# angelocatalani/neural-network-compression

Hardware: AMD Instinct MI355X
Metric: weights/sec through prune+k-means (K=256) (higher is better)
Workload: dtype f32

## Files before the change

neural_network_compression_amd/csrc/nnc_common.hpp:

```cpp
#pragma once
#include <hip/hip_runtime.h>
#include <hip/hip_ext.h>

#include <algorithm>
#include <atomic>
#include <chrono>
#include <mutex>
#include <cmath>
#include <cstdio>
#include <cstdlib>
#include <cstring>
#include <queue>
#include <string>
#include <vector>

#include "nnc.h"

int nnc_set_error_(int code, const char *msg);
int nnc_current_device_(void);
int nnc_cu_count_(void);
void nnc_prof_take_(int tag, hipEvent_t *a, hipEvent_t *b);

static inline int fail(int code, const std::string &msg) { return nnc_set_error_(code, msg.c_str()); }
static inline int current_device() { return nnc_current_device_(); }
static inline int cu_count() { return nnc_cu_count_(); }
static inline void prof_take(int tag, hipEvent_t *a, hipEvent_t *b) { nnc_prof_take_(tag, a, b); }
#define NNC_MAX_DEVICES 64

#define HIPCHK(expr)                                                                       \
    do {                                                                                   \
        hipError_t e_ = (expr);                                                            \
        if (e_ != hipSuccess)                                                              \
            return fail(NNC_EHIP, std::string(#expr) + ": " + hipGetErrorString(e_));      \
    } while (0)

#define LAUNCHCHK(name)                                                                    \
    do {                                                                                   \
        hipError_t e_ = hipGetLastError();                                                 \
        if (e_ != hipSuccess)                                                              \
            return fail(NNC_EHIP, std::string("launch ") + name + ": " + hipGetErrorString(e_)); \
    } while (0)

static inline hipStream_t S(void *stream) { return reinterpret_cast<hipStream_t>(stream); }

static inline int stream_grid(int64_t work_items, int threads, int per_cu)
{
    int64_t blocks = (work_items + threads - 1) / threads;
    int64_t cap = (int64_t)cu_count() * per_cu;
    if (blocks < 1) blocks = 1;
    return (int)std::min<int64_t>(blocks, cap);
}

#define NNC_LAUNCH_PROF(tag, kernel, grid, block, lds, stream, ...)                                   \
    do {                                                                                               \
        hipEvent_t ea_, eb_;                                                                           \
        prof_take(tag, &ea_, &eb_);                                                                    \
        hipExtLaunchKernelGGL(kernel, grid, block, lds, stream, ea_, eb_, 0, __VA_ARGS__);             \
    } while (0)

#define WAVE 64

__device__ __forceinline__ void wave_lds_fence()
{
    __builtin_amdgcn_fence(__ATOMIC_RELEASE, "wavefront");
    __builtin_amdgcn_wave_barrier();
    __builtin_amdgcn_fence(__ATOMIC_ACQUIRE, "wavefront");
}

#define LEAF 128
struct PwHeap { int start[256]; int len[256]; float val[256]; };


template <bool WAVE_ONLY = false, typename F>
__device__ float block_pairwise_sum(F elem, int n, PwHeap *hp)
{
    const int tid = threadIdx.x, nthr = blockDim.x;
    if (n <= LEAF) {
        if (tid < 8) {
            float res = 0.0f;
            if (n < 8) {
                for (int i = 0; i < n; i++) res += elem(i);
            } else {
                float r = elem(tid);
                const int lim = n - (n % 8);
                for (int i = 8; i < lim; i += 8) r += elem(i + tid);
                r = r + __shfl_xor(r, 1);
                r = r + __shfl_xor(r, 2);
                r = r + __shfl_xor(r, 4);
                res = r;
                for (int i = lim; i < n; i++) res += elem(i);
            }
            if (tid == 0) hp->val[1] = res;
        }
        if (WAVE_ONLY) wave_lds_fence();
        else __syncthreads();
        return hp->val[1];
    }
    for (int i = tid; i < 256; i += nthr) { hp->start[i] = 0; hp->len[i] = 0; hp->val[i] = 0.0f; }
    __syncthreads();
    if (tid == 0) { hp->start[1] = 0; hp->len[1] = n; }
    __syncthreads();
    int depth = 0;
    while (depth < 7 && ((n + (1 << depth) - 1) >> depth) > LEAF) depth++;
    if (depth < 7) depth++;
    for (int lev = 0; lev < depth; lev++) {
        const int i = (1 << lev) + tid;
        if (tid < (1 << lev)) {
            const int l = hp->len[i];
            if (l > LEAF) {
                int n2 = l / 2; n2 -= n2 % 8;
                hp->start[2 * i] = hp->start[i]; hp->len[2 * i] = n2;
                hp->start[2 * i + 1] = hp->start[i] + n2; hp->len[2 * i + 1] = l - n2;
            }
        }
        __syncthreads();
    }
    const int j = tid & 7;
    for (int node = 1 + (tid >> 3); node < (2 << depth) && node < 256; node += (nthr >> 3)) {
        const int l = hp->len[node];
        if (l > 0 && l <= LEAF) {
            const int st = hp->start[node];
            float res;
            if (l < 8) {
                res = 0.0f;
                for (int i = 0; i < l; i++) res += elem(st + i);
            } else {
                float r = elem(st + j);
                const int lim = l - (l % 8);
                for (int i = 8; i < lim; i += 8) r += elem(st + i + j);
                r = r + __shfl_xor(r, 1);
                r = r + __shfl_xor(r, 2);
                r = r + __shfl_xor(r, 4);
                res = r;
                for (int i = lim; i < l; i++) res += elem(st + i);
            }
            if (j == 0) hp->val[node] = res;
        }
    }
    __syncthreads();
    for (int lev = depth - 1; lev >= 0; lev--) {
        const int i = (1 << lev) + tid;
        if (tid < (1 << lev) && hp->len[i] > LEAF) hp->val[i] = hp->val[2 * i] + hp->val[2 * i + 1];
        __syncthreads();
    }
    return hp->val[1];
}

template <typename F>
__device__ float wave_pairwise_sum(F elem, int n, PwHeap *hp)
{
    const int lane = threadIdx.x & 63;
    if (n <= LEAF) {
        if (lane < 8) {
            float res = 0.0f;
            if (n < 8) {
                for (int i = 0; i < n; i++) res += elem(i);
            } else {
                float r = elem(lane);
                const int lim = n - (n % 8);
                for (int i = 8; i < lim; i += 8) r += elem(i + lane);
                r = r + __shfl_xor(r, 1);
                r = r + __shfl_xor(r, 2);
                r = r + __shfl_xor(r, 4);
                res = r;
                for (int i = lim; i < n; i++) res += elem(i);
            }
            if (lane == 0) hp->val[1] = res;
        }
        wave_lds_fence();
        return hp->val[1];
    }
    hp->start[lane] = 0; hp->len[lane] = 0; hp->val[lane] = 0.0f;
    wave_lds_fence();
    if (lane == 0) { hp->start[1] = 0; hp->len[1] = n; }
    wave_lds_fence();
    int depth = 0;
    while (depth < 5 && ((n + (1 << depth) - 1) >> depth) > LEAF) depth++;
    if (depth < 5) depth++;
    for (int lev = 0; lev < depth; lev++) {
        const int i = (1 << lev) + lane;
        if (lane < (1 << lev)) {
            const int l = hp->len[i];
            if (l > LEAF) {
                int n2 = l / 2; n2 -= n2 % 8;
                hp->start[2 * i] = hp->start[i]; hp->len[2 * i] = n2;
                hp->start[2 * i + 1] = hp->start[i] + n2; hp->len[2 * i + 1] = l - n2;
            }
        }
        wave_lds_fence();
    }
    const int j8 = lane & 7;
    for (int node = 1 + (lane >> 3); node < (2 << depth) && node < 64; node += 8) {
        const int l = hp->len[node];
        if (l > 0 && l <= LEAF) {
            const int st = hp->start[node];
            float res;
            if (l < 8) {
                res = 0.0f;
                for (int i = 0; i < l; i++) res += elem(st + i);
            } else {
                float r = elem(st + j8);
                const int lim = l - (l % 8);
                for (int i = 8; i < lim; i += 8) r += elem(st + i + j8);
                r = r + __shfl_xor(r, 1);
                r = r + __shfl_xor(r, 2);
                r = r + __shfl_xor(r, 4);
                res = r;
                for (int i = lim; i < l; i++) res += elem(st + i);
            }
            if (j8 == 0) hp->val[node] = res;
        }
    }
    wave_lds_fence();
    for (int lev = depth - 1; lev >= 0; lev--) {
        const int i = (1 << lev) + lane;
        if (lane < (1 << lev) && hp->len[i] > LEAF) hp->val[i] = hp->val[2 * i] + hp->val[2 * i + 1];
        wave_lds_fence();
    }
    return hp->val[1];
}
```

neural_network_compression_amd/csrc/nnc_hip.hip:

```cpp
#include "nnc_common.hpp"
#include "nnc_km_shared.hpp"


extern "C" size_t nnc_kmeans_workspace_bytes(int32_t k)
{
    (void)k;
    return sizeof(KmWs) + 256;
}

extern "C" int32_t nnc_fix_shift(float absmax, int64_t n_total)
{
    int L = 1;
    while (((int64_t)1 << L) < n_total && L < 62) L++;
    if (!(absmax > 0.0f) || !std::isfinite(absmax)) return 0;
    int P = 0;
    (void)std::frexp((double)absmax, &P);
    return std::min(28, 62 - L) - P;
}

__device__ __forceinline__ int fix_f32(float v, int Sft)
{
    return (int)rintf(ldexpf(v, Sft));
}

// ... 230 lines not shown
    if (MODE == 1 && n_dev) n = *n_dev;
    unsigned long long *trace = (MODE == 0) ? NNC_KM_TRACE_PTR : nullptr;
    unsigned long long tr0 = 0, tr1 = 0, tr2 = 0;
    if (trace) tr0 = __builtin_amdgcn_s_memrealtime();

    const int64_t nvec = VEC ? (n >> 2) : 0;
    const int64_t nsteps = nvec / KM_THREADS;
    const int64_t tails = DEAL ? (int64_t)(gridDim.x >> 1) : 0;
    const int64_t nmain = nsteps - 2 * tails;
    const int64_t per = (nmain + gridDim.x - 1) / gridDim.x;
    int64_t s0 = tails + (int64_t)blockIdx.x * per;
    const int64_t mend = nsteps - tails;
    if (s0 > mend) s0 = mend;
    const int64_t s1 = (s0 + per < mend) ? (s0 + per) : mend;
    const int64_t dealt = DEAL ? (((int64_t)blockIdx.x < tails) ? (int64_t)blockIdx.x : nsteps - 1 - ((int64_t)blockIdx.x - tails)) : 0;
    const int64_t count = (s1 - s0) + (DEAL ? 1 : 0);
    auto step_of = [&](int64_t kk) -> int64_t { return DEAL ? (kk == 0 ? dealt : s0 + kk - 1) : s0 + kk; };
    const float4 *x4 = reinterpret_cast<const float4 *>(x);
    const float4 *base = x4 + threadIdx.x;
#ifdef KM_NT_LOADS
    auto ld = [&](int64_t kk) -> float4 { return kk < count ? __builtin_nontemporal_load(&base[step_of(kk) * KM_THREADS]) : make_float4(0.f, 0.f, 0.f, 0.f); };
#else
    auto ld = [&](int64_t kk) -> float4 { return kk < count ? base[step_of(kk) * KM_THREADS] : make_float4(0.f, 0.f, 0.f, 0.f); };
#endif
    float4 r[KM_RING];
#pragma unroll
    for (int j = 0; j < KM_RING; j++) r[j] = ld(j);

    if (MODE == 0 && !(which & 2) && (ws->st.done | ws->st.paused)) return;
    if (MODE == 1 && n_dev && s0 >= s1 && blockIdx.x != gridDim.x - 1) return;
    const int k = ws->p.k;
    const int glog2 = ws->glog2, rlog2 = ws->rlog2;
    const int G = 1 << glog2;
    const int kp = (k + 7) & ~7;
    const int t = ws->cur ^ (which & 1);
    const KmTab *__restrict__ tab = &ws->tab[t];
#ifdef KM_KU_FAST
    const int kt = (which & 1) ? tab->ku : ws->ku_cur;
#else
    const int kt = tab->ku;
#endif

    uint16_t *cell_s = reinterpret_cast<uint16_t *>(smem);
    float4 *pair_s = reinterpret_cast<float4 *>(smem + ((size_t)2 << glog2));
    float *cval_s = reinterpret_cast<float *>(smem + ((size_t)2 << glog2) + (size_t)kp * 16);
    uint16_t *orig_s = reinterpret_cast<uint16_t *>(smem + ((size_t)2 << glog2) + (size_t)kp * 20);
    size_t off = (((size_t)2 << glog2) + (size_t)kp * 22 + 15) & ~(size_t)15;
    unsigned *ovf_s = reinterpret_cast<unsigned *>(smem + off);
    off += KM_OVF_MAX * 4;
    unsigned long long *sum_s = reinterpret_cast<unsigned long long *>(smem + off);
    unsigned *cnt_s = reinterpret_cast<unsigned *>(smem + off + ((size_t)k << rlog2) * 8);

    {
        const uint4 *src = reinterpret_cast<const uint4 *>(tab->cell);
        uint4 *dst = reinterpret_cast<uint4 *>(cell_s);
        for (int i = threadIdx.x; i < (G >> 3); i += KM_THREADS) dst[i] = src[i];
        for (int i = threadIdx.x; i < kt; i += KM_THREADS) {
            float2 a = tab->cand[i];
            float2 b = (i + 1 < kt) ? tab->cand[i + 1] : a;
            pair_s[i] = make_float4(a.x, a.y, b.x, b.y);
            cval_s[i] = a.x;
            orig_s[i] = tab->orig[i];
        }
        {
            const int novf = min(tab->n_ovf, KM_OVF_MAX);
            for (int i = threadIdx.x; i < novf; i += KM_THREADS) ovf_s[i] = tab->ovf[i];
        }
        if (MODE == 0) {
            const int tot = k << rlog2;
            for (int i = threadIdx.x; i < tot; i += KM_THREADS) { sum_s[i] = 0ull; cnt_s[i] = 0u; }
        }
        if (MODE == 1 && dist_hist) {
            unsigned *hz = reinterpret_cast<unsigned *>(sum_s);
            for (int i = threadIdx.x; i < 4096; i += KM_THREADS) hz[i] = 0u;
        }
    }
    __syncthreads();
    unsigned *hist_s = (MODE == 1 && dist_hist) ? reinterpret_cast<unsigned *>(sum_s) : nullptr;
    KmHistRun hr;
    hr.bin = 0xFFFFFFFFu; hr.cnt = 0;

    KmCtx c;
    c.cell_s = cell_s; c.pair_s = pair_s; c.cval_s = cval_s; c.orig_s = orig_s; c.ovf_s = ovf_s; c.sum_s = sum_s; c.cnt_s = cnt_s;
    c.mean = ws->p.x_mean; c.lo = ws->p.lo; c.inv = ws->inv;
    c.Sft = ws->p.fix_shift; c.gmax = G - 1; c.k = kt; c.rlog2 = rlog2;
    c.rep = threadIdx.x & ((1 << rlog2) - 1);
    KmRun run;
    run.p = -1; run.cnt = 0; run.sum = 0;
    if (trace) tr1 = __builtin_amdgcn_s_memrealtime();

    for (int64_t kk = 0; kk < count; kk += KM_RING) {
#pragma unroll
        for (int j = 0; j < KM_RING; j++) {
            const int64_t kcur = kk + j;
            const float4 v = r[j];
            r[j] = ld(kcur + KM_RING);
            if (kcur < count) {
                if (MODE == 0) km_accumulate4<ABL>(c, v, run);
                else {
                    const float xa[4] = {v.x, v.y, v.z, v.w};
                    km_emit<4, LT>(c, xa, 4 * (step_of(kcur) * KM_THREADS + threadIdx.x), labels_out, quant_out, dist_out, hist_s, hr);
                }
            }
        }
    }
    if (blockIdx.x == gridDim.x - 1) {
        const int64_t vdone = nsteps * KM_THREADS;
        {
            for (int64_t v = vdone + threadIdx.x; v < nvec; v += KM_THREADS) {
                const float4 a4 = x4[v];
                const float xa[4] = {a4.x, a4.y, a4.z, a4.w};
                if (MODE == 0) km_accumulate4<ABL>(c, a4, run);
                else km_emit<4, LT>(c, xa, 4 * v, labels_out, quant_out, dist_out, hist_s, hr);
            }
            for (int64_t i = (nvec << 2) + threadIdx.x; i < n; i += KM_THREADS) {
                const float xs[1] = {x[i]};
                if (MODE == 0) km_accumulate<1, ABL>(c, xs, run);
                else km_emit<1, LT>(c, xs, i, labels_out, quant_out, dist_out, hist_s, hr);
            }
        }
    }
    if (trace) tr2 = __builtin_amdgcn_s_memrealtime();
    if (MODE == 0) {
        if (ABL != 1 && ABL != 3) km_run_flush(c, run);
        else if (run.sum == 0x7fffffffffffll) sum_s[0] = run.sum;
        km_flush(c, ws);
    }
    if (MODE == 1 && hist_s) {
        if (hr.cnt) atomicAdd(&hist_s[hr.bin], hr.cnt);
        __syncthreads();
        for (int i = threadIdx.x; i < 4096; i += KM_THREADS)
            if (hist_s[i]) atomicAdd(&dist_hist[i], (unsigned long long)hist_s[i]);
    }
    if (trace && threadIdx.x == 0) {
        trace[4 * blockIdx.x + 0] = tr0; trace[4 * blockIdx.x + 1] = tr1;
        trace[4 * blockIdx.x + 2] = tr2; trace[4 * blockIdx.x + 3] = __builtin_amdgcn_s_memrealtime();
    }
}




#ifdef NNC_DIAG
#define KBSTAMP(slot, val) do { if (NNC_KM_TRACE_PTR && lane == 0) { NNC_KM_TRACE_PTR[(slot)] = __builtin_amdgcn_s_memrealtime(); } } while (0)
#else
#define KBSTAMP(slot, val) do { } while (0)
#endif
#define KM_PB NNC_PREFIX_BLOCK
#define KM_PG 1024
#define KM_TILE 2048
#ifndef KM_FIT_LAG
#define KM_FIT_LAG 2
#endif
#define KM_ZONE_REACH 12
#define KM_ACC_W 256
__host__ __device__ __forceinline__ int km_tile_len(int ncand) { int t = (2 * KM_TILE / (ncand < 2 ? 2 : ncand)) & ~63; return t < 64 ? 64 : t; }
#define KM_Q_VALID (1ull << 62)
#ifndef KM_PUBLISH_TILES
#define KM_PUBLISH_TILES 5
#endif


#define KM_DPP(v, ctrl) __builtin_amdgcn_update_dpp(0, (v), (ctrl), 0xF, 0xF, true)
#define KM_DPP_XOR1 0xB1
#define KM_DPP_XOR2 0x4E
#define KM_DPP_HMIRROR 0x141
#define KM_DPP_MIRROR 0x140
template <int CTRL> __device__ __forceinline__ long long km_dpp_ll(long long v)
{
    const int lo = KM_DPP((int)v, CTRL), hi = KM_DPP((int)(v >> 32), CTRL);
    return (long long)(((unsigned long long)(unsigned)hi << 32) | (unsigned long long)(unsigned)lo);
}
__device__ __forceinline__ long long km_readlane_ll(long long v, int l)
{
    const int lo = __builtin_amdgcn_readlane((int)v, l), hi = __builtin_amdgcn_readlane((int)(v >> 32), l);
    return (long long)(((unsigned long long)(unsigned)hi << 32) | (unsigned long long)(unsigned)lo);
}
__device__ __forceinline__ long long wave_sum_ll(long long v)
{
    v += km_dpp_ll<KM_DPP_XOR1>(v); v += km_dpp_ll<KM_DPP_XOR2>(v); v += km_dpp_ll<KM_DPP_HMIRROR>(v); v += km_dpp_ll<KM_DPP_MIRROR>(v);
    return (km_readlane_ll(v, 0) + km_readlane_ll(v, 16)) + (km_readlane_ll(v, 32) + km_readlane_ll(v, 48));
}
__device__ __forceinline__ double wave_max_d(double v)
{
    v = fmax(v, __longlong_as_double(km_dpp_ll<KM_DPP_XOR1>(__double_as_longlong(v))));
    v = fmax(v, __longlong_as_double(km_dpp_ll<KM_DPP_XOR2>(__double_as_longlong(v))));
    v = fmax(v, __longlong_as_double(km_dpp_ll<KM_DPP_HMIRROR>(__double_as_longlong(v))));
    v = fmax(v, __longlong_as_double(km_dpp_ll<KM_DPP_MIRROR>(__double_as_longlong(v))));
    const long long b = __double_as_longlong(v);
    return fmax(fmax(__longlong_as_double(km_readlane_ll(b, 0)), __longlong_as_double(km_readlane_ll(b, 16))),
                fmax(__longlong_as_double(km_readlane_ll(b, 32)), __longlong_as_double(km_readlane_ll(b, 48))));
}
__device__ __forceinline__ double wave_min_d(double v)
{
    v = fmin(v, __longlong_as_double(km_dpp_ll<KM_DPP_XOR1>(__double_as_longlong(v))));
    v = fmin(v, __longlong_as_double(km_dpp_ll<KM_DPP_XOR2>(__double_as_longlong(v))));
    v = fmin(v, __longlong_as_double(km_dpp_ll<KM_DPP_HMIRROR>(__double_as_longlong(v))));
    v = fmin(v, __longlong_as_double(km_dpp_ll<KM_DPP_MIRROR>(__double_as_longlong(v))));
    const long long b = __double_as_longlong(v);
    return fmin(fmin(__longlong_as_double(km_readlane_ll(b, 0)), __longlong_as_double(km_readlane_ll(b, 16))),
                fmin(__longlong_as_double(km_readlane_ll(b, 32)), __longlong_as_double(km_readlane_ll(b, 48))));
}
__device__ __forceinline__ int wave_max_i(int v)
{
    v = max(v, KM_DPP(v, KM_DPP_XOR1)); v = max(v, KM_DPP(v, KM_DPP_XOR2)); v = max(v, KM_DPP(v, KM_DPP_HMIRROR)); v = max(v, KM_DPP(v, KM_DPP_MIRROR));
    return max(max(__builtin_amdgcn_readlane(v, 0), __builtin_amdgcn_readlane(v, 16)), max(__builtin_amdgcn_readlane(v, 32), __builtin_amdgcn_readlane(v, 48)));
}

__host__ __device__ __forceinline__ long long km_prefix_nblk(long long n) { return (n + NNC_PREFIX_BLOCK - 1) / NNC_PREFIX_BLOCK; }
__device__ __forceinline__ const long long *km_pgrp(const long long *pblk, long long n) { return pblk + km_prefix_nblk(n) + 2; }
#define KL_BLK 64
__host__ __device__ __forceinline__ long long km_prefix_ngroups(long long n) { return (km_prefix_nblk(n) + 1 + KM_PG - 1) / KM_PG; }
__host__ __device__ __forceinline__ long long km_pfine_off(long long n) { return km_prefix_nblk(n) + 2 + km_prefix_ngroups(n) + 2; }

__device__ __forceinline__ long long km_prefix_at(const float *__restrict__ xs, const long long *__restrict__ pblk, long long r,
                                                  long long n, float mean, int Sft, int lane)
{
    const long long blk = r >> 8, base = blk << 8;
    const int rem = (int)(r - base);
    long long acc = 0;
    if (rem > 0) {
        const long long i0 = base + 4 * lane;
        if (base + KM_PB <= n) {
            const float4 v = *reinterpret_cast<const float4 *>(xs + i0);
            const int left = rem - 4 * lane;
            if (left > 0) acc += fix_f32(v.x - mean, Sft);
            if (left > 1) acc += fix_f32(v.y - mean, Sft);
            if (left > 2) acc += fix_f32(v.z - mean, Sft);
            if (left > 3) acc += fix_f32(v.w - mean, Sft);
        } else {
            for (int u = 0; u < 4; u++) if (i0 + u < r) acc += fix_f32(xs[i0 + u] - mean, Sft);
        }
        acc = wave_sum_ll(acc);
    }
    return pblk[blk] + km_pgrp(pblk, n)[blk / KM_PG] + acc;
}

struct KmPfx { float4 v; long long pb; int rem; };
__device__ __forceinline__ KmPfx km_prefix_load(const float *__restrict__ xs, const long long *__restrict__ pblk, long long r, long long n, int lane)
{
    KmPfx p;
    const long long blk = r >> 8, base = blk << 8;
    p.rem = (int)(r - base);
    p.pb = pblk[blk] + km_pgrp(pblk, n)[blk / KM_PG];
    p.v = make_float4(0.0f, 0.0f, 0.0f, 0.0f);
    if (p.rem > 0) {
        const long long i0 = base + 4 * lane;
        if (base + KM_PB <= n) p.v = *reinterpret_cast<const float4 *>(xs + i0);
        else {
            if (i0 + 0 < r) p.v.x = xs[i0 + 0];
            if (i0 + 1 < r) p.v.y = xs[i0 + 1];
            if (i0 + 2 < r) p.v.z = xs[i0 + 2];
            if (i0 + 3 < r) p.v.w = xs[i0 + 3];
        }
    }
    return p;
}
__device__ __forceinline__ long long km_prefix_finish(const KmPfx &p, float mean, int Sft, int lane)
{
    long long acc = 0;
    if (p.rem > 0) {
        const int left = p.rem - 4 * lane;
        if (left > 0) acc += fix_f32(p.v.x - mean, Sft);
        if (left > 1) acc += fix_f32(p.v.y - mean, Sft);
        if (left > 2) acc += fix_f32(p.v.z - mean, Sft);
        if (left > 3) acc += fix_f32(p.v.w - mean, Sft);
        acc = wave_sum_ll(acc);
    }
    return p.pb + acc;
}

__device__ __forceinline__ void km_shard_add(KmWs *ws, int p, long long sum, unsigned long long cnt)
{
    if (cnt) {
        atomicAdd(reinterpret_cast<unsigned long long *>(&ws->shard_sum[p & (KM_NSHARD - 1)][p]), (unsigned long long)sum);
        atomicAdd(&ws->shard_cnt[p & (KM_NSHARD - 1)][p], cnt);
    }
}

__device__ __forceinline__ void km_bounds_range(const float *__restrict__ xs, long long s, long long e, int plo, int phi, const KmTab *__restrict__ tab,
                                                        KmWs *ws, float mean, int Sft, int lane)
{
    s = uni_ll(s); e = uni_ll(e); plo = uni_i(plo); phi = uni_i(phi);
    const bool chk = e - s >= 128 && phi > plo;
    float x0 = 0.0f, x1 = 1.0f;
    if (chk) { x0 = xs[s]; x1 = xs[e - 1]; }
    auto flat_run = [&]() {
        const float xc = x0 - mean;
        float bestd = INFINITY;
        int best = plo, besto = 0x7fffffff;
        for (int c = plo; c <= phi; c++) {
            const float2 cm = tab->cand[c];
            const int oc = (int)tab->orig[c];
            const float d = cm.y + (-2.0f * (xc * cm.x));
            if (d < bestd || (d == bestd && oc < besto)) { bestd = d; best = c; besto = oc; }
        }
        if (lane == 0) km_shard_add(ws, best, (long long)fix_f32(xc, Sft) * (e - s), (unsigned long long)(e - s));
    };
    if (phi <= plo) {
        long long sum = 0;
        unsigned cnt = 0;
        for (long long i = s + lane; i < e; i += 64) { sum += fix_f32(xs[i] - mean, Sft); cnt++; }
        sum = wave_sum_ll(sum);
        const long long c = wave_sum_ll((long long)cnt);
        if (lane == 0) km_shard_add(ws, plo, sum, (unsigned long long)c);
        return;
// ... 492 lines not shown
        __syncthreads();
        if (tid == 0) carry_s += tot;
        __syncthreads();
    }
    if (tid == 0) pgrp[ngroups] = carry_s;
}


__device__ __forceinline__ double km_rcp_up(double d)
{
    const float r = __frcp_rn((float)d);
    return (d > 1e-37 && d < 1e37) ? (double)r * (1.0 + 9.5367431640625e-07) : 1.0 / d;
}

struct KmZone { double lo, hi; };
__device__ __forceinline__ KmZone km_pair_zone(const double cp, const double cq, const double xb)
{
    const double U = 5.9604644775390625e-08;
    const double delta = cq - cp;
    const double cm = fmax(fabs(cp), fabs(cq));
    const double mid = 0.5 * (cp + cq);
    const double E = 2.5 * U * (cm * cm + 2.0 * xb * cm) + 1e-42;
    const double w0 = E * km_rcp_up(delta);
    KmZone z;
    z.lo = mid - w0; z.hi = mid + w0;
    const double S = fabs(cp) + fabs(cq);
    const double den = 2.0 * delta - 4.5 * U * S;
    if (den > delta) {
        const float cpf = (float)cp, cqf = (float)cq;
        const double Cp = (double)(cpf * cpf), Cq = (double)(cqf * cqf);
        const double d2 = 2.0 * delta;
        double xs;
        if (d2 > 1e-37 && d2 < 1e37) {
            const double r0 = (double)__frcp_rn((float)d2);
            xs = (Cq - Cp) * (r0 * (2.0 - d2 * r0));
        } else xs = (Cq - Cp) / d2;
        const double Ds = fmax(fabs(Cp - 2.0 * xs * cp), fabs(Cq - 2.0 * xs * cq));
        const double num = U * (2.0 * Ds + 2.0000005 * fabs(xs) * S) * 1.000001 + 1e-42;
        const double w = (num * km_rcp_up(den)) * 1.000001 + fabs(xs) * 1e-13;
        z.lo = fmax(z.lo, xs - w); z.hi = fmin(z.hi, xs + w);
    }
    return z;
}
__device__ __forceinline__ double km_pair_slack(const double delta, const double xb) { return 1.25e-7 * xb * xb * km_rcp_up(delta); }

__device__ __forceinline__ void km_lds_barrier() { asm volatile("s_waitcnt lgkmcnt(0)\n\ts_barrier\n\ts_waitcnt lgkmcnt(0)" ::: "memory"); }
__device__ __forceinline__ unsigned f32_ordered_bits(float x)
{
    const unsigned u = __float_as_uint(x);
    return (u & 0x80000000u) ? ~u : (u | 0x80000000u);
}
__device__ __forceinline__ float f32_from_ordered_bits(unsigned o)
{
    return __uint_as_float((o & 0x80000000u) ? (o & 0x7FFFFFFFu) : ~o);
}

#include "nnc_lloyd.hpp"

__device__ __forceinline__ int km_vote_or(int *word, const int x)
{
    if (__any(x) && (threadIdx.x & 63) == 0) *word = 1;
    km_lds_barrier();
    return *word;
}
__device__ __forceinline__ int km_vote_count(int *word, const int x)
{
    const int c = (int)__popcll(__ballot(x != 0));
    if (c && (threadIdx.x & 63) == 0) atomicAdd(word, c);
    km_lds_barrier();
    return *word;
}

template <int NT, bool MASS>
__device__ int km_finalize_relocate(KmWs *__restrict__ ws, const float *__restrict__ xs, const long long n, const KmTab *__restrict__ tab, const int ku,
                                    const int k, const int cur, long long *sum_o, long long *cnt_o, const float mean, const int Sft)
{
    constexpr int KC = NNC_KMAX;
    __shared__ __align__(16) unsigned char buf[sizeof(KlHead) + (size_t)KC * (8 + 8 + 4 + 4 + 4 + 4 + 2 + 2) + 4096 * 2];
    KlHead *hd = reinterpret_cast<KlHead *>(buf);
    KlArr L = {};
    {
        unsigned char *q = buf + sizeof(KlHead);
        L.A = reinterpret_cast<long long *>(q); q += (size_t)KC * 8;
        L.B = reinterpret_cast<long long *>(q); q += (size_t)KC * 8;
        L.cs = reinterpret_cast<float *>(q); q += (size_t)KC * 4;
        L.csq = reinterpret_cast<float *>(q); q += (size_t)KC * 4;
        L.cold = reinterpret_cast<float *>(q); q += (size_t)KC * 4;
        L.call = reinterpret_cast<float *>(q); q += (size_t)KC * 4;
        L.so = reinterpret_cast<uint16_t *>(q); q += (size_t)KC * 2;
        L.phi = reinterpret_cast<uint16_t *>(q); q += (size_t)KC * 2;
        L.qj = reinterpret_cast<uint16_t *>(q);
    }
    const int tid = threadIdx.x;
    if (tid == 0) { hd->n_empty = 0; hd->ku = ku; hd->nch = 0; hd->slow = 0; hd->r_flat = 0; }
    __syncthreads();
    int e = 0;
    for (int j = tid; j < k; j += NT) { e += cnt_o[j] == 0; L.cold[j] = ws->c[cur][j]; }
    if (e) atomicAdd(&hd->n_empty, e);
    __syncthreads();
    const bool mass = MASS && hd->n_empty > KL_RM_MAX;
    if (!MASS && hd->n_empty > KL_RM_MAX) return 0;
    if (!mass && 2 * ku > KL_RPASS * (NT / 8)) return 0;
    for (int p = tid; p < ku; p += NT) {
        const float2 c = tab->cand[p];
        L.cs[p] = c.x; L.csq[p] = c.y; L.so[p] = tab->orig[p];
        L.A[p] = ws->hint_a[p]; L.B[p] = ws->hint_b[p];
        const int ph = ws->bnd_phi[p];
        L.phi[p] = (uint16_t)(ph < p + 1 ? p + 1 : (ph > ku - 1 ? ku - 1 : ph));
    }
    __syncthreads();
    int *qfirst = reinterpret_cast<int *>(L.call);
    for (int j = tid; j + 1 < ku; j += NT) {
        const long long bm = j > 0 ? L.B[j - 1] : 0, a = L.A[j], b = L.B[j];
        const long long s0 = a > bm ? a : bm;
        const long long len = b - s0;
        qfirst[j] = 0;
        if (len > 0) {
            const int cs_ = (int)L.phi[j] == j + 1 ? KL_CHUNK : KL_CHUNK_CROWD;
            const long long nc = (len + cs_ - 1) / cs_;
            if (nc > (mass ? 512 : 64)) hd->slow = 1;
            else {
                const int first = atomicAdd(&hd->nch, (int)nc);
                qfirst[j] = first;
                for (int i = 0; i < (int)nc; i++) if (first + i < KL_QMAX) L.qj[first + i] = (uint16_t)j;
            }
        }
    }
    __syncthreads();
    if (NNC_FIN_TRACE_PTR && tid == 0) {
        unsigned long long *rt = NNC_FIN_TRACE_PTR;
        const int it = min(ws->st.iter, 63);
        rt[300 + 4 * it] = (unsigned long long)hd->n_empty; rt[301 + 4 * it] = (unsigned long long)hd->nch; rt[302 + 4 * it] = (unsigned long long)hd->slow; rt[303 + 4 * it] = (unsigned long long)ku;
    }
    if (hd->slow || hd->nch > 1024) return 0;
    if constexpr (MASS) {
        if (mass) {
            __shared__ KlMass mass_s;
            return kl_relocate_mass<NT>(xs, n, ws, hd, L, &mass_s, sum_o, cnt_o, k, hd->nch, mean, Sft);
        }
    }
    return kl_relocate<NT>(xs, n, ws, hd, L, sum_o, cnt_o, k, hd->nch, mean, Sft);
}

template <int NT, bool ONEWAVE, bool MASS = false>
__device__ __forceinline__ bool km_finalize_body(KmWs *__restrict__ ws, int mode, int resume, int *gcell, int *hcell, int *ku_out, const bool lazy = false,
                                                 const float *__restrict__ reloc_xs = nullptr, const long long reloc_n = 0, const int k_hint = 0)
{
    static_assert(!ONEWAVE || NT == 64, "the barrier-free form is for a single wave");
#define FIN_SYNC() do { if (ONEWAVE) wave_lds_fence(); else km_lds_barrier(); } while (0)
#define FIN_OR(slot, x) (ONEWAVE ? (int)__any(x) : km_vote_or(&fin_votes[slot], (x)))
#define FIN_AND(slot, x) (ONEWAVE ? (int)__all(x) : !km_vote_or(&fin_votes[slot], !(x)))
#define FIN_COUNT(slot, x) (ONEWAVE ? (int)__popcll(__ballot(x)) : km_vote_count(&fin_votes[slot], (x)))
    __shared__ int fin_votes[8];
    __shared__ long long sum_o[NNC_KMAX];
    __shared__ long long cnt_o[NNC_KMAX];
    __shared__ __align__(16) float cnew[NNC_KMAX];
    __shared__ float cs[NNC_KMAX];
    __shared__ uint16_t so[NNC_KMAX];
    __shared__ float sq[NNC_KMAX];
    __shared__ unsigned long long sh_key;
    __shared__ int ovf_n;
    __shared__ PwHeap heap;
    __shared__ float cu[NNC_KMAX];
    __shared__ uint16_t sou[NNC_KMAX];
    __shared__ double wave_a[NT / 64], wave_b[NT / 64];

    const int tid = threadIdx.x;
    unsigned long long *ftr = NNC_FIN_TRACE_PTR;
#define FSTAMP(i) do { if (ftr && tid == 0) ftr[i] = __builtin_amdgcn_s_memrealtime(); } while (0)
    FSTAMP(0);
    if (tid == 0) ws->cells_pending = 0;
    if (!ONEWAVE && tid < 8) fin_votes[tid] = 0;
    const int kb = k_hint > 0 ? min(k_hint, (int)NNC_KMAX) : (int)NNC_KMAX;
    const bool takes_a_pass = mode != FIN_FROM_PARTIALS;
    const bool from_shards = mode == FIN_FROM_SHARDS || mode == FIN_PACK_ONLY;
    const int qn_raw = takes_a_pass ? ws->q_n : 0;
    const int st_done = ws->st.done, st_paused = ws->st.paused, st_iter = ws->st.iter, reloc_fail = ws->reloc_fail;
    const int spec_go = ws->spec_go;
    const int k = ws->p.k, Sft = ws->p.fix_shift, max_iter = ws->p.max_iter, glog2 = ws->glog2;
    const float tol_v = ws->p.tol, p_lo = ws->p.lo, p_hi = ws->p.hi, inv_f = ws->inv;
    const long long n_tot = ws->p.n_total;
    const int ku0 = ws->tab[0].ku, ku1 = ws->tab[1].ku;
    int cur = ws->cur;
    const bool track = (mode == FIN_FROM_SHARDS) || (mode == FIN_FROM_PARTIALS && !resume);
    constexpr int RR = 2;
    long long pc[RR];
    float c_both[RR][2];
    uint16_t pm_both[RR][2], pmn_both[RR][2];
#pragma unroll
    for (int r = 0; r < RR; r++) {
        pc[r] = 0; c_both[r][0] = c_both[r][1] = 0.0f; pm_both[r][0] = pm_both[r][1] = pmn_both[r][0] = pmn_both[r][1] = 0;
        const int j = tid + r * NT;
        if (j < kb) {
            if (track) pc[r] = ws->prev_counts[j];
            if (mode != FIN_INIT) {
                c_both[r][0] = ws->c[0][j]; c_both[r][1] = ws->c[1][j];
                pm_both[r][0] = ws->tab[0].perm[j]; pm_both[r][1] = ws->tab[1].perm[j];
                if (j + 1 < NNC_KMAX) { pmn_both[r][0] = ws->tab[0].perm[j + 1]; pmn_both[r][1] = ws->tab[1].perm[j + 1]; }
            }
        }
    }
    long long sh_s[KM_NSHARD];
    unsigned long long sh_c[KM_NSHARD];
    uint16_t og_both[2] = {0, 0};
    const bool sh_pre = from_shards && tid < kb;
#pragma unroll
    for (int sh = 0; sh < KM_NSHARD; sh++) { sh_s[sh] = 0; sh_c[sh] = 0; }
    if (sh_pre) {
        og_both[0] = ws->tab[0].orig[tid]; og_both[1] = ws->tab[1].orig[tid];
#pragma unroll
        for (int sh = 0; sh < KM_NSHARD; sh++) { sh_s[sh] = ws->shard_sum[sh][tid]; sh_c[sh] = ws->shard_cnt[sh][tid]; }
    }
    const int qn = min(qn_raw, (int)NNC_KMAX);
    for (int r = tid; r < qn; r += NT) { ws->q_w0[r] = 0ull; ws->q_w1[r] = 0ull; ws->q_next[r] = 0; }
    FSTAMP(44);
#define FIN_QUEUE_RESET() do { if (tid == 0 && takes_a_pass) { ws->q_n = 0; ws->q_searched = 0; ws->help_hint = qn > 0; } } while (0)
#define FIN_LEAVE() do { if (ONEWAVE) wave_lds_fence(); else __syncthreads(); FIN_QUEUE_RESET(); return false; } while (0)
    if (mode != FIN_INIT && mode != FIN_PACK_ONLY && st_done) FIN_LEAVE();
    if (mode == FIN_FROM_SHARDS && st_paused) FIN_LEAVE();
    if (mode == FIN_PACK_ONLY && (st_done | st_paused)) {
        const int k2 = 2 * k;
        for (int i = tid; i < k2; i += NT) ws->partials[i] = ws->partials_local[i];
        FIN_LEAVE();
    }
    if (mode == FIN_FROM_PARTIALS && st_paused && !resume) FIN_LEAVE();
    if (resume == 2 && !spec_go) FIN_LEAVE();
    if (resume && reloc_fail) {
        if (tid == 0) ws->st.paused = 2;
        FIN_LEAVE();
    }

    float cold_r[RR];
    int spa[RR], spb[RR];
#pragma unroll
    for (int r = 0; r < RR; r++) {
        const int j = tid + r * NT;
        const bool in = mode != FIN_INIT && j < k;
        cold_r[r] = in ? (cur ? c_both[r][1] : c_both[r][0]) : 0.0f;
        spa[r] = in ? (int)(cur ? pm_both[r][1] : pm_both[r][0]) : 0;
        spb[r] = (in && j + 1 < k) ? (int)(cur ? pmn_both[r][1] : pmn_both[r][0]) : 0;
        if (!(track && j < k)) pc[r] = 0;
    }
    if (from_shards) {
        const KmTab *tab = &ws->tab[cur];
        const int ku_cur = cur ? ku1 : ku0;
        for (int j = tid; j < k; j += NT) { sum_o[j] = 0; cnt_o[j] = 0; }
        FIN_SYNC();
        FIN_QUEUE_RESET();
        FSTAMP(45);
        for (int p = tid; p < ku_cur; p += NT) {
            long long s = 0;
            unsigned long long c = 0;
            int o;
            if (p == tid && sh_pre) {
                o = cur ? og_both[1] : og_both[0];
#pragma unroll
                for (int sh = 0; sh < KM_NSHARD; sh++) { s += sh_s[sh]; c += sh_c[sh]; }
            } else {
                o = tab->orig[p];
                for (int sh = 0; sh < KM_NSHARD; sh++) { s += ws->shard_sum[sh][p]; c += ws->shard_cnt[sh][p]; }
            }
            for (int sh = 0; sh < KM_NSHARD; sh++) { ws->shard_sum[sh][p] = 0; ws->shard_cnt[sh][p] = 0; }
            sum_o[o] = s; cnt_o[o] = (long long)c;
        }
        FIN_SYNC();
        FSTAMP(46);
        for (int j = tid; j < k; j += NT) {
            ws->partials[j] = sum_o[j]; ws->partials[k + j] = cnt_o[j];
            ws->partials_local[j] = sum_o[j]; ws->partials_local[k + j] = cnt_o[j];
        }
        if (mode == FIN_PACK_ONLY) return false;
    } else if (mode == FIN_FROM_PARTIALS) {
        for (int j = tid; j < k; j += NT) { sum_o[j] = ws->partials[j]; cnt_o[j] = ws->partials[k + j]; }
    }
    FIN_SYNC();
    FSTAMP(47);
    if (!from_shards) FIN_QUEUE_RESET();
    int same_counts_now = 0;
    bool settled_event = false;
    if (track) {
        int count_diff = 0;
#pragma unroll
        for (int r = 0; r < RR; r++) {
            const int j = tid + r * NT;
            if (j < k) {
                const long long c = cnt_o[j];
                count_diff |= (pc[r] != c);
                ws->prev_counts[j] = c;
            }
        }
        const int any_diff = FIN_OR(0, count_diff);
        same_counts_now = any_diff ? 0 : 1;
        if (tid == 0) ws->st.same_counts = any_diff ? 0 : 1;
    }
    FSTAMP(1);

    if (mode != FIN_INIT) {
        int my_empty = 0;
        for (int j = tid; j < k; j += NT) my_empty += (cnt_o[j] == 0);
        if (tid == 0) sh_key = 0ull;
        int n_empty = FIN_COUNT(1, my_empty);
        bool settled = false;
        settled_event = false;
        if constexpr (!ONEWAVE) {
            if (n_empty > 0 && (MASS || n_empty <= KL_RM_MAX) && !resume && reloc_xs && mode == FIN_FROM_SHARDS && lazy && !(st_iter >= 1 && same_counts_now)) {
                __syncthreads();
                if (ftr && tid == 0) { ftr[20] = ftr[0]; ftr[21] = __builtin_amdgcn_s_memrealtime(); }
                const KmTab *tabc = &ws->tab[cur];
                settled = km_finalize_relocate<NT, MASS>(ws, reloc_xs, reloc_n, tabc, cur ? ku1 : ku0, k, cur, sum_o, cnt_o, ws->p.x_mean, Sft) != 0;
                if (settled) { n_empty = 0; settled_event = true; }
                if (settled && ftr && tid == 0) ftr[22] = __builtin_amdgcn_s_memrealtime();
            }
        }
        if (n_empty > 0 && !resume) {
            int tot_empty = 0;
            if (tid == 0) {
                for (int j = 0; j < k; j++) tot_empty += (cnt_o[j] == 0);
                ws->st.paused = 1; ws->st.n_empty = tot_empty;
                if (lazy) ws->tab[cur].n_ovf = 0;
            }
            return false;
        }
        for (int j = tid; j < k; j += NT)
            if (cnt_o[j] > 0) cnew[j] = (float)ldexp((double)sum_o[j] / (double)cnt_o[j], -Sft);
        FIN_SYNC();
        if (n_empty > 0) {
            for (int j = tid; j < k; j += NT)
                atomicMax(&sh_key, ((unsigned long long)cnt_o[j] << 11) | (unsigned long long)(2047 - j));
            FIN_SYNC();
            const int amax = 2047 - (int)(sh_key & 2047ull);
            for (int j = tid; j < k; j += NT)
                if (cnt_o[j] <= 0) {
                    cnew[j] = (amax < j) ? cnew[amax] : (float)ldexp((double)sum_o[amax], -Sft);
                }
            FIN_SYNC();
        }
        FSTAMP(2);
#pragma unroll
        for (int r = 0; r < RR; r++) {
            const int j = tid + r * NT;
            if (j < k) {
                float d = cnew[j] - cold_r[r];
                float s2 = d * d;
                float sft = (float)sqrt((double)s2);
                sq[j] = sft * sft;
            }
        }
        FIN_SYNC();
        float tot = 0.0f;
        if (ONEWAVE) tot = block_pairwise_sum<true>([&](int i) { return sq[i]; }, k, &heap);
        else if (tid < 64) tot = wave_pairwise_sum([&](int i) { return sq[i]; }, k, &heap);
        if (tid == 0) {
            int iter = st_iter + 1;
            int done = 0;
            if (tot <= tol_v) done = 1;
            else if (iter >= max_iter) done = 2;
            ws->st.iter = iter; ws->st.shift_tot = tot; ws->st.done = done;
            ws->st.paused = 0; ws->st.n_empty = 0;
            ws->cur = cur ^ 1;
        }
        cur ^= 1;
        for (int j = tid; j < k; j += NT) ws->c[cur][j] = cnew[j];
        FIN_SYNC();
    } else {
        for (int j = tid; j < k; j += NT) cnew[j] = ws->c[cur][j];
        FIN_SYNC();
    }

    FSTAMP(3);
    KmTab *tab = &ws->tab[cur];
    int still_sorted = 0;
    if (mode != FIN_INIT) {
        int ok = 1;
#pragma unroll
        for (int r = 0; r < RR; r++) {
            const int p = tid + r * NT;
            if (p < k) {
                const int a = spa[r];
                so[p] = (uint16_t)a;
                cs[p] = cnew[a];
                if (p + 1 < k) {
                    const int b = spb[r];
                    const float va = cnew[a], vb = cnew[b];
                    ok &= (va < vb) || (va == vb && a < b);
                }
            }
        }
        FSTAMP(12);
        still_sorted = FIN_AND(2, ok);
        const bool moved_far = resume || settled_event;
        for (int pass = 0; pass < 3 && !still_sorted && !moved_far; pass++) {
            for (int parity = 0; parity < 2; parity++) {
                for (int p = 2 * tid + parity; p + 1 < k; p += 2 * NT) {
                    const float va = cs[p], vb = cs[p + 1];
                    const uint16_t a = so[p], b = so[p + 1];
                    if (!((va < vb) || (va == vb && a < b))) { cs[p] = vb; cs[p + 1] = va; so[p] = b; so[p + 1] = a; }
                }
                FIN_SYNC();
            }
            int ok2 = 1;
            for (int p = tid; p + 1 < k; p += NT) {
                const float va = cs[p], vb = cs[p + 1];
                ok2 &= (va < vb) || (va == vb && so[p] < so[p + 1]);
            }
            still_sorted = FIN_AND(3 + pass, ok2);
        }
    }
    FSTAMP(8);
    if (ftr && tid == 0) ftr[13] = (unsigned long long)still_sorted;
    if (!still_sorted) {
        int parts = 1;
        while (parts < 64 && k * parts * 2 <= NT) parts <<= 1;
        const int per_part = (((k + parts - 1) / parts) + 3) & ~3;
        const float4 *c4 = reinterpret_cast<const float4 *>(cnew);
        for (int t = tid; t < ((k * parts + NT - 1) / NT) * NT; t += NT) {
            const int j = t / parts, part = t % parts;
            int rank = 0;
            float v = 0.0f;
            if (j < k) {
                v = cnew[j];
                const int i0 = part * per_part, i1 = min(k, i0 + per_part);
#pragma unroll 4
                for (int i = i0; i < i1; i += 4) {
                    const float4 u = c4[i >> 2];
                    rank += (int)(u.x < v) | ((int)(u.x == v) & (int)(i < j));
                    rank += ((int)(u.y < v) | ((int)(u.y == v) & (int)(i + 1 < j))) & (int)(i + 1 < i1);
                    rank += ((int)(u.z < v) | ((int)(u.z == v) & (int)(i + 2 < j))) & (int)(i + 2 < i1);
                    rank += ((int)(u.w < v) | ((int)(u.w == v) & (int)(i + 3 < j))) & (int)(i + 3 < i1);
                }
            }
            for (int off = 1; off < parts; off <<= 1) rank += __shfl_xor(rank, off);
            if (j < k && part == 0) { cs[rank] = v; so[rank] = (uint16_t)j; }
        }
    }
    FIN_SYNC();
    FSTAMP(9);
    if (settled_event && ftr && tid == 0) { ftr[23] = ftr[3]; ftr[24] = ftr[9]; }
    int ku = 0;
    {
        int *wave_i = reinterpret_cast<int *>(wave_a);
        const int rounds_u = (k + NT - 1) / NT;
        int carry = 0;
        for (int rd = 0; rd < rounds_u; rd++) {
            const int p = rd * NT + tid;
            float v = 0.0f;
            int o = 0, first = 0;
            if (p < k) {
                v = cs[p]; o = so[p];
                tab->perm[p] = (uint16_t)o;
                first = (p == 0) || (cs[p - 1] != v);
            }
            const unsigned long long bal = __ballot(first);
            const int before = __popcll(bal & ((1ull << (tid & 63)) - 1ull));
            if ((tid & 63) == 0) wave_i[tid >> 6] = __popcll(bal);
            FIN_SYNC();
            int pre = carry, tot = carry;
            for (int w = 0; w < NT / 64; w++) { const int wv = wave_i[w]; if (w < (tid >> 6)) pre += wv; tot += wv; }
            if (first) { cu[pre + before] = v; sou[pre + before] = (uint16_t)o; }
            carry = tot;
            FIN_SYNC();
        }
        ku = min(carry, k);
    }
    FSTAMP(10);
    for (int p = tid; p < ku; p += NT) {
        const float v = cu[p];
        cs[p] = v;
        tab->cand[p] = make_float2(v, v * v);
        tab->orig[p] = sou[p];
        ws->bnd.cand[p] = make_float2(v, v * v);
        ws->bnd.orig[p] = sou[p];
    }
    if (tid == 0) { tab->ku = ku; ws->ku_cur = ku; ws->bnd.ku = ku; ovf_n = 0; }
    FIN_SYNC();
    FSTAMP(4);
    const double U = 5.9604644775390625e-08;
    const double xb = fmax(fabs((double)p_lo), fabs((double)p_hi));
    const int G = 1 << glog2;
    const double lo = (double)p_lo;
    const double inv = (double)inv_f;
    const double ra = inv > 0.0 ? (1.0 - 4.0 * U) / inv * (1.0 - 4.0 * U) : 0.0;
    const double rb = inv > 0.0 ? (1.0 + 4.0 * U) / inv * (1.0 + 4.0 * U) : 0.0;
    {
        const int rounds = (ku + NT - 1) / NT;
        int *wave_i = reinterpret_cast<int *>(wave_a);
        int carry_g = -2;
        int wide_zone = 0;
        double *zhi = reinterpret_cast<double *>(sum_o), *zlo = reinterpret_cast<double *>(cnt_o);
        const int zd = ku > 0 ? max(1, min(min(4, NT / max(ku, 1)), NNC_KMAX / max(ku, 1))) : 1;
        for (int t = tid; t < zd * ku; t += NT) {
            const int d = t / ku, p = t - d * ku, q = p + d + 1;
            if (q < ku) {
                const KmZone z = km_pair_zone((double)cs[p], (double)cs[q], xb);
                zhi[d * ku + p] = z.hi; zlo[d * ku + q] = z.lo;
            }
        }
        FSTAMP(13);
        FIN_SYNC();
        FSTAMP(14);
        for (int rd = 0; rd < rounds; rd++) {
            const int p = rd * NT + tid;
            int gp = -2, hp_ = G + 1;
            if (p < ku) {
                const double cp = (double)cs[p];
                double right = p + 1 < ku ? zhi[p] : INFINITY, left = p > 0 ? zlo[p] : -INFINITY;
                for (int q = p + 2; q < ku && q - p <= KM_ZONE_REACH; q++) {
                    const double cq = (double)cs[q];
                    const double mid = 0.5 * (cp + cq);
                    const double delta = cq - cp;
                    if (mid - km_pair_slack(delta, xb) >= right) break;
                    const int d = q - p - 1;
                    if (delta > 0.0) right = fmin(right, d < zd ? zhi[d * ku + p] : km_pair_zone(cp, cq, xb).hi);
                }
                for (int q = p - 2; q >= 0 && p - q <= KM_ZONE_REACH; q--) {
                    const double cq = (double)cs[q];
                    const double mid = 0.5 * (cp + cq);
                    const double delta = cp - cq;
                    if (mid + km_pair_slack(delta, xb) <= left) break;
                    const int d = p - q - 1;
                    if (delta > 0.0) left = fmax(left, d < zd ? zlo[d * ku + p] : km_pair_zone(cq, cp, xb).lo);
                }
                tab->zl[p] = left; tab->zr[p] = right;
                ws->bnd.zl[p] = left; ws->bnd.zr[p] = right;
                if (p + 1 < ku && (zhi[p] - zlo[p + 1]) * (double)n_tot * 4.0 > 16.0 * (double)KM_TILE * ((double)p_hi - (double)p_lo)) wide_zone = 1;
                gp = G - 1; hp_ = 0;
                if (inv > 0.0 && !lazy) {
                    const double qa = (right - lo) / ra;
                    gp = (qa >= (double)(G - 1)) ? (G - 1) : (qa < 0.0 ? -1 : (int)(qa * (1.0 + 1e-12)));
                    if (gp > G - 1) gp = G - 1;
                    const double qb = ((left - lo) / rb - 1.0) * (1.0 - 1e-12);
                    if (qb <= 0.0) hp_ = 0;
                    else if (qb >= (double)G) hp_ = G;
                    else { hp_ = (int)qb; if ((double)hp_ < qb) hp_++; }
                }
            }
            if (p < ku) { gcell[p] = gp; hcell[p] = hp_; }
        }
        FSTAMP(15);
        const bool placed = mode == FIN_INIT || resume || settled_event;
        if (FIN_OR(6, wide_zone) && tid == 0 && placed) ws->help_hint = 2;
        FIN_SYNC();
        FSTAMP(11);
        if (settled_event && ftr && tid == 0) ftr[25] = ftr[11];
        if (!lazy) {
        int *wave_g = reinterpret_cast<int *>(wave_a);
        int *wave_h = reinterpret_cast<int *>(wave_b);
        int carry_h = G + 1;
        const int lane = tid & 63, myw = tid >> 6;
        for (int it = 0; it < rounds; it++) {
            const int rg = it, rh = rounds - 1 - it;
            int a = (rg * NT + tid < ku) ? gcell[rg * NT + tid] : -2;
            int b = (rh * NT + tid < ku) ? hcell[rh * NT + tid] : G + 1;
            for (int off = 1; off < 64; off <<= 1) {
                const int oa = __shfl_up(a, off), ob = __shfl_down(b, off);
                if (lane >= off) a = max(a, oa);
                if (lane + off < 64) b = min(b, ob);
            }
            if (lane == 63) wave_g[myw] = a;
            if (lane == 0) wave_h[myw] = b;
            FIN_SYNC();
            int pre = carry_g, totg = carry_g, suf = carry_h, toth = carry_h;
            for (int w = 0; w < NT / 64; w++) {
                const int gv = wave_g[w], hv = wave_h[w];
// ... 1867 lines not shown
```

Baseline: 10.26 billion.

## Add partial re-rank of moved centroids in finalize and compute pairwise tree ranges arithmetically

When the finalize kernel's centroids are no longer sorted after a resume or settled event, it now tries a partial re-rank. Centroids that were previously empty, or that sit next to an inversion, are marked as movers. If every other centroid is still in order and there are at most 32 movers, only the movers are ranked against the rest and scattered into place, skipping the full O(k^2) rank sort. Separately, wave_pairwise_sum now derives each tree node's start and length by bit-walking instead of building the heap in LDS with fences. The cost is extra shared memory, an atomic counter per mover, and a new flag written to kl_stats.

```diff
diff --git a/neural_network_compression_amd/csrc/nnc_common.hpp b/neural_network_compression_amd/csrc/nnc_common.hpp
--- a/neural_network_compression_amd/csrc/nnc_common.hpp
+++ b/neural_network_compression_amd/csrc/nnc_common.hpp
@@ -146,6 +146,17 @@
     return hp->val[1];
 }
 
+__device__ __forceinline__ void pw_node_range(const int node, const int n, int &start, int &len)
+{
+    start = 0; len = n;
+    for (int b = 30 - __clz(node); b >= 0; b--) {
+        if (len > LEAF) {
+            int n2 = len / 2; n2 -= n2 % 8;
+            if ((node >> b) & 1) { start += n2; len -= n2; } else len = n2;
+        } else len = 0;
+    }
+}
+
 template <typename F>
 __device__ float wave_pairwise_sum(F elem, int n, PwHeap *hp)
 {
@@ -170,30 +181,14 @@
         wave_lds_fence();
         return hp->val[1];
     }
-    hp->start[lane] = 0; hp->len[lane] = 0; hp->val[lane] = 0.0f;
-    wave_lds_fence();
-    if (lane == 0) { hp->start[1] = 0; hp->len[1] = n; }
-    wave_lds_fence();
     int depth = 0;
     while (depth < 5 && ((n + (1 << depth) - 1) >> depth) > LEAF) depth++;
     if (depth < 5) depth++;
-    for (int lev = 0; lev < depth; lev++) {
-        const int i = (1 << lev) + lane;
-        if (lane < (1 << lev)) {
-            const int l = hp->len[i];
-            if (l > LEAF) {
-                int n2 = l / 2; n2 -= n2 % 8;
-                hp->start[2 * i] = hp->start[i]; hp->len[2 * i] = n2;
-                hp->start[2 * i + 1] = hp->start[i] + n2; hp->len[2 * i + 1] = l - n2;
-            }
-        }
-        wave_lds_fence();
-    }
     const int j8 = lane & 7;
     for (int node = 1 + (lane >> 3); node < (2 << depth) && node < 64; node += 8) {
-        const int l = hp->len[node];
+        int st, l;
+        pw_node_range(node, n, st, l);
         if (l > 0 && l <= LEAF) {
-            const int st = hp->start[node];
             float res;
             if (l < 8) {
                 res = 0.0f;
@@ -212,9 +207,11 @@
         }
     }
     wave_lds_fence();
+    int my_st, my_len = 0;
+    const int my_lev = 31 - __clz(lane | 1);
+    if (lane > 0) pw_node_range(lane, n, my_st, my_len);
     for (int lev = depth - 1; lev >= 0; lev--) {
-        const int i = (1 << lev) + lane;
-        if (lane < (1 << lev) && hp->len[i] > LEAF) hp->val[i] = hp->val[2 * i] + hp->val[2 * i + 1];
+        if (lane > 0 && my_lev == lev && my_len > LEAF) hp->val[lane] = hp->val[2 * lane] + hp->val[2 * lane + 1];
         wave_lds_fence();
     }
     return hp->val[1];
diff --git a/neural_network_compression_amd/csrc/nnc_hip.hip b/neural_network_compression_amd/csrc/nnc_hip.hip
--- a/neural_network_compression_amd/csrc/nnc_hip.hip
+++ b/neural_network_compression_amd/csrc/nnc_hip.hip
@@ -406,6 +406,7 @@
 #ifndef KM_FIT_LAG
 #define KM_FIT_LAG 2
 #endif
+#define KM_MV_MAX 32
 #define KM_ZONE_REACH 12
 #define KM_ACC_W 256
 __host__ __device__ __forceinline__ int km_tile_len(int ncand) { int t = (2 * KM_TILE / (ncand < 2 ? 2 : ncand)) & ~63; return t < 64 ? 64 : t; }
@@ -1204,6 +1205,10 @@
 #define FIN_AND(slot, x) (ONEWAVE ? (int)__all(x) : !km_vote_or(&fin_votes[slot], !(x)))
 #define FIN_COUNT(slot, x) (ONEWAVE ? (int)__popcll(__ballot(x)) : km_vote_count(&fin_votes[slot], (x)))
     __shared__ int fin_votes[8];
+    __shared__ uint8_t mv[NNC_KMAX], mv_inv[NNC_KMAX];
+    __shared__ int mv_n, mv_rank[KM_MV_MAX];
+    __shared__ float mv_val[KM_MV_MAX];
+    __shared__ uint16_t mv_idx[KM_MV_MAX], mv_pos[KM_MV_MAX];
     __shared__ long long sum_o[NNC_KMAX];
     __shared__ long long cnt_o[NNC_KMAX];
     __shared__ __align__(16) float cnew[NNC_KMAX];
@@ -1223,6 +1228,8 @@
     FSTAMP(0);
     if (tid == 0) ws->cells_pending = 0;
     if (!ONEWAVE && tid < 8) fin_votes[tid] = 0;
+    if (!ONEWAVE && tid < KM_MV_MAX) mv_rank[tid] = 0;
+    if (!ONEWAVE && tid == 0) mv_n = 0;
     const int kb = k_hint > 0 ? min(k_hint, (int)NNC_KMAX) : (int)NNC_KMAX;
     const bool takes_a_pass = mode != FIN_FROM_PARTIALS;
     const bool from_shards = mode == FIN_FROM_SHARDS || mode == FIN_PACK_ONLY;
@@ -1244,7 +1251,7 @@
         pc[r] = 0; c_both[r][0] = c_both[r][1] = 0.0f; pm_both[r][0] = pm_both[r][1] = pmn_both[r][0] = pmn_both[r][1] = 0;
         const int j = tid + r * NT;
         if (j < kb) {
-            if (track) pc[r] = ws->prev_counts[j];
+            if (track || resume) pc[r] = ws->prev_counts[j];
             if (mode != FIN_INIT) {
                 c_both[r][0] = ws->c[0][j]; c_both[r][1] = ws->c[1][j];
                 pm_both[r][0] = ws->tab[0].perm[j]; pm_both[r][1] = ws->tab[1].perm[j];
@@ -1284,10 +1291,12 @@
 
     float cold_r[RR];
     int spa[RR], spb[RR];
+    bool was_empty[RR];
 #pragma unroll
     for (int r = 0; r < RR; r++) {
         const int j = tid + r * NT;
         const bool in = mode != FIN_INIT && j < k;
+        was_empty[r] = resume && in && pc[r] == 0;
         cold_r[r] = in ? (cur ? c_both[r][1] : c_both[r][0]) : 0.0f;
         spa[r] = in ? (int)(cur ? pm_both[r][1] : pm_both[r][0]) : 0;
         spb[r] = (in && j + 1 < k) ? (int)(cur ? pmn_both[r][1] : pmn_both[r][0]) : 0;
@@ -1338,6 +1347,7 @@
             if (j < k) {
                 const long long c = cnt_o[j];
                 count_diff |= (pc[r] != c);
+                was_empty[r] = c == 0;
                 ws->prev_counts[j] = c;
             }
         }
@@ -1396,6 +1406,7 @@
                 float s2 = d * d;
                 float sft = (float)sqrt((double)s2);
                 sq[j] = sft * sft;
+                if (!ONEWAVE) { mv[j] = was_empty[r] ? 1 : 0; mv_inv[j] = 0; }
             }
         }
         FIN_SYNC();
@@ -1460,7 +1471,92 @@
     }
     FSTAMP(8);
     if (ftr && tid == 0) ftr[13] = (unsigned long long)still_sorted;
-    if (!still_sorted) {
+    bool ranked = false;
+    if constexpr (!ONEWAVE) {
+        if (!still_sorted && mode != FIN_INIT && (resume || settled_event)) {
+            float v_r[RR];
+            int a_r[RR], slot_r[RR];
+            auto next_plain = [&](const int p, const bool with_inv) {
+                int q = p + 1;
+                while (q < k && q - p <= KM_MV_MAX && (mv[so[q]] || (with_inv && mv_inv[q]))) q++;
+                return (q < k && q - p <= KM_MV_MAX) ? q : k;
+            };
+#pragma unroll
+            for (int r = 0; r < RR; r++) {
+                const int p = tid + r * NT;
+                v_r[r] = 0.0f; a_r[r] = 0; slot_r[r] = -1;
+                if (p < k) {
+                    const float v = cs[p];
+                    const int a = so[p];
+                    v_r[r] = v; a_r[r] = a;
+                    if (!mv[a]) {
+                        const int q = next_plain(p, false);
+                        if (q < k) {
+                            const float vb = cs[q];
+                            const int b = so[q];
+                            if (!((v < vb) || (v == vb && a < b))) { mv_inv[p] = 1; mv_inv[q] = 1; }
+                        }
+                    }
+                }
+            }
+            FIN_SYNC();
+            int ok = 1;
+#pragma unroll
+            for (int r = 0; r < RR; r++) {
+                const int p = tid + r * NT;
+                if (p < k) {
+                    const float v = v_r[r];
+                    const int a = a_r[r];
+                    if (mv[a] || mv_inv[p]) {
+                        const int sl = atomicAdd(&mv_n, 1);
+                        slot_r[r] = sl;
+                        if (sl < KM_MV_MAX) { mv_val[sl] = v; mv_idx[sl] = (uint16_t)a; mv_pos[sl] = (uint16_t)p; }
+                    } else {
+                        const int q = next_plain(p, true);
+                        if (q < k) {
+                            const float vb = cs[q];
+                            const int b = so[q];
+                            ok &= (int)(v < vb) | ((int)(v == vb) & (int)(a < b));
+                        } else if (p + KM_MV_MAX + 1 < k) ok = 0;
+                    }
+                }
+            }
+            const int in_order = FIN_AND(7, ok);
+            const int m = mv_n;
+            if (in_order && m > 0 && m <= KM_MV_MAX) {
+                ranked = true;
+                int rank_r[RR];
+#pragma unroll
+                for (int r = 0; r < RR; r++) {
+                    const int p = tid + r * NT;
+                    rank_r[r] = p;
+                    if (r * NT < k) {
+                        int rank = p;
+                        for (int i = 0; i < m; i++) {
+                            const float u = mv_val[i];
+                            const int o = mv_idx[i], pos = mv_pos[i];
+                            const int lt = (int)(p < k) & ((int)(v_r[r] < u) | ((int)(v_r[r] == u) & (int)(a_r[r] < o)));
+                            rank += (1 - lt) - (int)(pos < p);
+                            const int c = (int)__popcll(__ballot(lt));
+                            if (c && (tid & 63) == 0) atomicAdd(&mv_rank[i], c);
+                        }
+                        rank_r[r] = rank;
+                    }
+                }
+                FIN_SYNC();
+#pragma unroll
+                for (int r = 0; r < RR; r++) {
+                    const int p = tid + r * NT;
+                    if (p < k) {
+                        const int rank = slot_r[r] >= 0 ? mv_rank[slot_r[r]] : rank_r[r];
+                        cs[rank] = v_r[r]; so[rank] = (uint16_t)a_r[r];
+                    }
+                }
+            }
+        }
+    }
+    if (!ONEWAVE && !still_sorted && mode != FIN_INIT && (resume || settled_event) && tid == 0) atomicOr(&ws->kl_stats[6], ranked ? 256 : 512);
+    if (!still_sorted && !ranked) {
         int parts = 1;
         while (parts < 64 && k * parts * 2 <= NT) parts <<= 1;
         const int per_part = (((k + parts - 1) / parts) + 3) & ~3;
```

After: 9.952 billion. 3.0% lower.
